# Sum02dean/GCN-STRING

Hardware: AMD Instinct MI355X
Metric: graphs/sec (fwd+bwd) on E.coli-sized batches; GCNConv SpMM achieved HBM GB/s (higher is better)
Workload: dtype f32; 1 GPU; config2: E. coli-shaped DisjointLoader batch, B=32 graphs per GPU, F=128, fp32, 2-layer GCNConv(relu)+GlobalSumPool+Dense softmax, CCE (from-logits form of tf.function), SGD; global_graphs=32, nodes_per_gpu=22576, nnz_per_gpu=333676, features=128, hidden=128, parallelism=dp1 (graphs sharded, RCCL all-reduce of 33284 fp32), hip_graph=False, gemm_precision=f32, cce=logits, activation_storage=fp32

## Files before the change

### gcn-string_amd/csrc/fused.hip

```cpp
#include "common.h"

namespace {

typedef float f32x4v __attribute__((ext_vector_type(4)));
typedef float f32x2 __attribute__((ext_vector_type(2)));
typedef __bf16 fbf16x8 __attribute__((ext_vector_type(8)));

constexpr int kFRows = 32;
constexpr int kFCap = 1024;

struct FusedArgs {
  const int32_t* rowptr; const int32_t* colidx; const float* vals;
  const float* x; int64_t ldx;
  int32_t n;
  const float* w; int32_t ldw;
  int32_t nc;
  const float* bias; int act;
  float* s; int64_t lds;
  float* wt_out;
  int w_t;
  float* out; int64_t ldo;
  const int32_t* node_graph; const int32_t* gp; const float* dp; int64_t lddp; int avg;
  const float* mask; int64_t ldmask;
  float* dz2; int64_t lddz2;
  float* colpart;
  float* tp_part; float* tp_cnt;
  const float* hd_part; const float* hd_cnt; int hd_rows; int hd_b;
  float* hd_psum; float* hd_csum;
  const float* hd_w; const float* hd_bias; const float* hd_y; int hd_c; float hd_denom; int hd_fl;
  unsigned char* m8_out; const unsigned char* m8; int64_t ldm8;
  int dbg;
};

__device__ __forceinline__ float4 fbuf4(__amdgpu_buffer_rsrc_t rs, unsigned off) {
  const f32x4v r = __builtin_bit_cast(f32x4v, __builtin_amdgcn_raw_buffer_load_b128(rs, off, 0, 0));
  return make_float4(r.x, r.y, r.z, r.w);
}
__device__ __forceinline__ float4 f4fma(float v, float4 h, float4 a) {
  const f32x2 w = {v, v};
  const f32x2 lo = __builtin_elementwise_fma(w, f32x2{h.x, h.y}, f32x2{a.x, a.y});
  const f32x2 hi = __builtin_elementwise_fma(w, f32x2{h.z, h.w}, f32x2{a.z, a.w});
  return make_float4(lo[0], lo[1], hi[0], hi[1]);
}
__device__ __forceinline__ float4 f4step(float4 a) {
  const f32x2 big = {0x1p127f, 0x1p127f};
  f32x2 lo = {a.x, a.y}, hi = {a.z, a.w}, t0, t1;
  asm("v_pk_mul_f32 %0, %1, %2" : "=v"(t0) : "v"(lo), "v"(big));
  asm("v_pk_mul_f32 %0, %1, %2" : "=v"(t1) : "v"(hi), "v"(big));
  asm("v_pk_mul_f32 %0, %1, %2 clamp" : "=v"(lo) : "v"(t0), "v"(big));
  asm("v_pk_mul_f32 %0, %1, %2 clamp" : "=v"(hi) : "v"(t1), "v"(big));
  return make_float4(lo[0], lo[1], hi[0], hi[1]);
}

constexpr int kM8B = 8;
constexpr int kM8U = 8;
typedef unsigned m8x2 __attribute__((ext_vector_type(2)));
template <int MLB> struct M8Bytes { typedef unsigned type; };
template <> struct M8Bytes<8> { typedef m8x2 type; };
template <int MLB>
__device__ __forceinline__ typename M8Bytes<MLB>::type m8load(__amdgpu_buffer_rsrc_t rs, unsigned off) {
  if constexpr (MLB == 8) return __builtin_bit_cast(m8x2, __builtin_amdgcn_raw_buffer_load_b64(rs, off, 0, 0));
  else if constexpr (MLB == 4) return (unsigned)__builtin_amdgcn_raw_buffer_load_b32(rs, off, 0, 0);
  else return (unsigned)(unsigned short)__builtin_amdgcn_raw_buffer_load_b16(rs, off, 0, 0);
}
template <int MLB>
__device__ __forceinline__ typename M8Bytes<MLB>::type m8own(const unsigned char* q) {
  if constexpr (MLB == 8) return *reinterpret_cast<const m8x2*>(q);
  else if constexpr (MLB == 4) return *reinterpret_cast<const unsigned*>(q);
  else return (unsigned)*reinterpret_cast<const unsigned short*>(q);
}
template <int MLB>
__device__ __forceinline__ unsigned m8word(typename M8Bytes<MLB>::type m, int d) {
  if constexpr (MLB == 8) return m[d]; else return m;
}
template <int MLB>
__device__ __forceinline__ void m8fma(float v, typename M8Bytes<MLB>::type m, float (&a)[MLB]) {
#pragma unroll
  for (int c = 0; c < MLB; ++c) a[c] = fmaf(v, (float)((m8word<MLB>(m, c / 4) >> (8 * (c % 4))) & 0xffu), a[c]);
}

__device__ __forceinline__ void f4acc(float4& a, const float4 q) { a.x += q.x; a.y += q.y; a.z += q.z; a.w += q.w; }

template <int LPR>
__device__ __forceinline__ float2 fused_head_dlogits(const FusedArgs& p, float4 pv, int rows, float4 w0, float4 w1, float b0,
                                                     float b1, float y0, float y1) {
  float sc = 1.0f;
  if (p.avg) { sc = 1.0f / (float)max(rows, 1); pv.x *= sc; pv.y *= sc; pv.z *= sc; pv.w *= sc; }
  const bool two = p.hd_c > 1;
  float z0 = fmaf(pv.w, w0.w, fmaf(pv.z, w0.z, fmaf(pv.y, w0.y, pv.x * w0.x)));
  float z1 = fmaf(pv.w, w1.w, fmaf(pv.z, w1.z, fmaf(pv.y, w1.y, pv.x * w1.x)));
#pragma unroll
  for (int off = 1; off < LPR; off <<= 1) { z0 += __shfl_xor(z0, off); z1 += __shfl_xor(z1, off); }
  z0 += b0;
  z1 = two ? z1 + b1 : -INFINITY;
  const float m = fmaxf(z0, z1), e0 = expf(z0 - m), e1 = expf(z1 - m), sum = e0 + e1;
  const float p0 = e0 / sum, p1 = e1 / sum;
  const bool k0 = p.hd_fl || (p0 > 1e-7f && p0 < 1.0f - 1e-7f), k1 = two && (p.hd_fl || (p1 > 1e-7f && p1 < 1.0f - 1e-7f));
  const float ymsum = (k0 ? y0 : 0.f) + (k1 ? y1 : 0.f);
  const float dl0 = (p0 * ymsum - (k0 ? y0 : 0.f)) / p.hd_denom, dl1 = two ? (p1 * ymsum - (k1 ? y1 : 0.f)) / p.hd_denom : 0.f;
  return make_float2(dl0 * sc, dl1 * sc);
}

template <int K, bool WEIGHTED, bool BWD, bool X3 = false, bool M8 = false>
__global__ __launch_bounds__(512, 6) void gcn_conv_fused_kernel(FusedArgs p) {
  constexpr int MLB = K / 16 < kM8B ? K / 16 : kM8B, UM = kM8U;
  typedef typename M8Bytes<MLB>::type m8v;
  constexpr int HL = K / 4;
  constexpr int LPR = M8 ? K / MLB : K / 4;
  constexpr int CPL = K / LPR;
  constexpr int GW = 64 / LPR;
  constexpr int NG = 8 * GW;
  constexpr int RPG = NG >= kFRows ? 1 : kFRows / NG;
  constexpr int U = 4;
  constexpr int SL = 2 * U;
  static_assert(UM <= SL, "the mask gather reads up to UM - 1 entries past a row's end");
  static_assert(K == 32 || K == 64 || K == 128, "gather width");
  static_assert(!M8 || (BWD && RPG == 1), "the byte-image gather is a backward form, one row per lane group");
  __shared__ __attribute__((aligned(16))) float tile[kFRows][K + 4];
  __shared__ __attribute__((aligned(8))) int2 s_ent[kFCap + SL];
  __shared__ int32_t s_rp[kFRows + 1];
  __shared__ unsigned char s_mb[BWD ? kFRows * 32 : 1];
  __shared__ float2 s_dl[BWD ? kFRows : 1];
  __shared__ __attribute__((aligned(16))) float s_w3[BWD ? 2 : 1][K];
  __shared__ float s_b3[2];
  __shared__ int32_t s_g[BWD ? 1 : kFRows];
  static_assert(!BWD || sizeof(float) * kFRows * (K + 4) >= sizeof(float4) * 2 * 8 * 2 * HL, "the head's wave partials alias the tile");
#ifdef GCNX_TUNING
  const int dbg = p.dbg;
#else
  constexpr int dbg = 0;
#endif

  const int tid = threadIdx.x, lane = tid & 63, wave = tid >> 6;
  const int ntiles = gridDim.x;
  const int t = gcnx_xcd_remap(blockIdx.x, ntiles);
  const int r0 = t * kFRows, nr = min(p.n - r0, kFRows);
  if (tid <= nr) s_rp[tid] = p.rowptr[r0 + tid];
  if (!BWD && p.tp_part && tid < kFRows)
    s_g[tid] = tid < nr ? min(max(p.node_graph[r0 + tid], 0), p.hd_b - 1) : -1;
  const int e0 = p.rowptr[r0], e1 = p.rowptr[r0 + nr];
  const int staged = min(e1 - e0, kFCap);
  const unsigned ld4 = M8 ? (unsigned)p.ldm8 : (unsigned)p.ldx * 4u;
  for (int i = tid; i < staged + SL; i += 512) {
    int2 en = make_int2(0, 0);
    if (i < staged) {
      en.x = (int)((unsigned)p.colidx[e0 + i] * ld4);
      en.y = WEIGHTED ? __float_as_int(p.vals[e0 + i]) : 0x3f800000;
    }
    s_ent[i] = en;
  }
  const int gid = wave * GW + lane / LPR, sub = lane % LPR;
  const __amdgpu_buffer_rsrc_t xr =
      __builtin_amdgcn_make_buffer_rsrc(M8 ? (void*)p.m8 : (void*)p.x, (short)0, (int)((unsigned)p.n * ld4), 0x00020000);
  int grow[RPG];
  if (BWD) {
#pragma unroll
    for (int j = 0; j < RPG; ++j) {
      const int r = gid + j * NG;
      grow[j] = (r < nr && gid < kFRows) ? p.node_graph[r0 + r] : -1;
    }
  }
  float4 mrow[2];
  const int mlanes = p.nc >> 2;
  if (BWD) {
#pragma unroll
    for (int q = 0; q < 2; ++q) {
      const int i = tid + 512 * q, row = i / mlanes, c4 = i - row * mlanes;
      mrow[q] = make_float4(0.f, 0.f, 0.f, 0.f);
      if (row < nr && !(dbg & 16)) mrow[q] = *reinterpret_cast<const float4*>(p.mask + (int64_t)(r0 + row) * p.ldmask + 4 * c4);
    }
  }
  float4 (*s_pv)[2][2][HL] = reinterpret_cast<float4 (*)[2][2][HL]>(&tile[0][0]);
  const int hsel = lane / HL, hsub = lane % HL;
  int g_first = 0;
  if (BWD && p.hd_part) {
    g_first = min(max(__builtin_amdgcn_readfirstlane(p.node_graph[r0]), 0), p.hd_b - 1);
    const int g_last = min(max(__builtin_amdgcn_readfirstlane(p.node_graph[r0 + nr - 1]), g_first), min(g_first + kFRows, p.hd_b) - 1);
    for (int i = tid; i < 2 * K; i += 512) {
      const int cls = i / K, k = i - cls * K;
      s_w3[cls][k] = cls < p.hd_c ? p.hd_w[(int64_t)k * p.hd_c + cls] : 0.f;
    }
    if (tid >= 2 * K && tid < 2 * K + 2) s_b3[tid - 2 * K] = (p.hd_bias && tid - 2 * K < p.hd_c) ? p.hd_bias[tid - 2 * K] : 0.f;
    const unsigned bytes = (unsigned)p.hd_rows * (unsigned)K * 4u;
    const __amdgpu_buffer_rsrc_t pr = __builtin_amdgcn_make_buffer_rsrc((void*)p.hd_part, (short)0, (int)bytes, 0x00020000);
    const __amdgpu_buffer_rsrc_t cr = __builtin_amdgcn_make_buffer_rsrc((void*)p.hd_cnt, (short)0, (int)bytes, 0x00020000);
    for (int gb = g_first; gb <= g_last; gb += 2) {
      if (gb > g_first) __syncthreads();
      int hd_g = 0, hd_n = 0;
      bool hd_desig = false;
      float y0 = 0.f, y1 = 0.f;
      if (hsel < 2) {
        hd_g = min(gb + hsel, g_last);
        const int hd_a = p.gp[hd_g];
        hd_n = p.gp[hd_g + 1] - hd_a;
        hd_desig = hd_a >= r0 && hd_n > 0;
        const int tlo = hd_a / kFRows, thi = hd_n > 0 ? (hd_a + hd_n - 1) / kFRows : tlo - 1;
        float4 ps = make_float4(0.f, 0.f, 0.f, 0.f), pc = ps;
        for (int tb = tlo + wave; __builtin_amdgcn_ballot_w64(tb <= thi) != 0; tb += 32) {
          float4 q[4], c[4];
#pragma unroll
          for (int u = 0; u < 4; ++u) {
            const int tt = tb + 8 * u;
            const unsigned off = tt <= thi ? ((unsigned)(tt + hd_g) * (unsigned)K + (unsigned)hsub * 4u) * 4u : 0xFFFFFFF0u;
            q[u] = fbuf4(pr, off);
            c[u] = fbuf4(cr, hd_desig ? off : 0xFFFFFFF0u);
          }
#pragma unroll
          for (int u = 0; u < 4; ++u) { f4acc(ps, q[u]); f4acc(pc, c[u]); }
        }
        s_pv[wave][0][hsel][hsub] = ps;
        s_pv[wave][1][hsel][hsub] = pc;
        if (wave == 0) {
          y0 = p.hd_y[(int64_t)hd_g * p.hd_c];
          y1 = p.hd_c > 1 ? p.hd_y[(int64_t)hd_g * p.hd_c + 1] : 0.f;
        }
      }
      __syncthreads();
      if (wave == 0 && hsel < 2) {
        float4 pv = make_float4(0.f, 0.f, 0.f, 0.f), pc = pv;
#pragma unroll 2
        for (int w = 0; w < 8; ++w) { f4acc(pv, s_pv[w][0][hsel][hsub]); f4acc(pc, s_pv[w][1][hsel][hsub]); }
        if (hd_desig) {
          *reinterpret_cast<float4*>(p.hd_psum + (int64_t)hd_g * K + hsub * 4) = pv;
          *reinterpret_cast<float4*>(p.hd_csum + (int64_t)hd_g * K + hsub * 4) = pc;
        }
        const float2 dl = fused_head_dlogits<HL>(p, pv, hd_n, *reinterpret_cast<const float4*>(&s_w3[0][hsub * 4]),
                                                  *reinterpret_cast<const float4*>(&s_w3[1][hsub * 4]),
                                                  s_b3[0], s_b3[1], y0, y1);
        if (hsub == 0) s_dl[hd_g - g_first] = dl;
      }
    }
  } else {
    __syncthreads();
  }
  if (BWD) {
#pragma unroll
    for (int q = 0; q < 2; ++q) {
      const int i = tid + 512 * q, row = i / mlanes, c4 = i - row * mlanes;
      if (row < kFRows)
        s_mb[row * 32 + c4] = (unsigned char)((mrow[q].x > 0.f ? 1u : 0u) | (mrow[q].y > 0.f ? 2u : 0u) | (mrow[q].z > 0.f ? 4u : 0u) |
                                              (mrow[q].w > 0.f ? 8u : 0u));
    }
  }
  float4 acc[RPG];
  int ea[RPG], eb[RPG], ebf[RPG];
  int len = 0;
#pragma unroll
  for (int j = 0; j < RPG; ++j) {
    const int r = gid + j * NG;
    acc[j] = make_float4(0.f, 0.f, 0.f, 0.f);
    const bool live = r < nr && gid < kFRows;
    ea[j] = live ? s_rp[r] - e0 : 0;
    eb[j] = live ? s_rp[r + 1] - e0 : 0;
    ebf[j] = min(eb[j], kFCap);
    ea[j] = min(ea[j], kFCap);
    len = max(len, ebf[j] - ea[j]);
  }
  if (dbg & 1) len = 0;
  const unsigned sub16 = (unsigned)sub * 16u;
  float am[M8 ? CPL : 1] = {};
  if constexpr (M8) {
    const unsigned subb = (unsigned)sub * (unsigned)MLB;
    for (int tt = 0; __builtin_amdgcn_ballot_w64(tt < len) != 0; tt += UM) {
      m8v hv[UM];
      float wv[UM];
      const int eb_ = min(ea[0] + tt, ebf[0]);
#pragma unroll
      for (int u = 0; u < UM; ++u) {
        const int e = eb_ + u;
        const int2 en = s_ent[e];
        wv[u] = __int_as_float(en.y);
        hv[u] = m8load<MLB>(xr, e < ebf[0] ? (unsigned)en.x + subb : 0xFFFFFFF0u);
      }
      __builtin_amdgcn_sched_barrier(0);
#pragma unroll
      for (int u = 0; u < UM; ++u) {
        m8fma<MLB>(wv[u], hv[u], am);
        if (u + 1 < UM) asm volatile("" : "+v"(hv[u + 1]), "+v"(am[0]));
      }
    }
    if (e1 - e0 > kFCap) {
      for (int e = max(eb[0] > 0 ? s_rp[gid] - e0 : 0, kFCap); e < eb[0]; ++e) {
        const float v = WEIGHTED ? p.vals[e0 + e] : 1.0f;
        m8fma<MLB>(v, m8load<MLB>(xr, (unsigned)p.colidx[e0 + e] * ld4 + subb), am);
      }
    }
  } else {
  for (int tt = 0; __builtin_amdgcn_ballot_w64(tt < len) != 0; tt += U) {
    float4 hv[RPG][U];
    float wv[RPG][U];
#pragma unroll
    for (int j = 0; j < RPG; ++j) {
      const int eb_ = min(ea[j] + tt, ebf[j]);
#pragma unroll
      for (int u = 0; u < U; ++u) {
        const int e = eb_ + u;
        const int2 en = s_ent[e];
        wv[j][u] = __int_as_float(en.y);
        hv[j][u] = fbuf4(xr, e < ebf[j] ? (unsigned)en.x + sub16 : 0xFFFFFFF0u);
      }
    }
    __builtin_amdgcn_sched_barrier(0);
#pragma unroll
    for (int j = 0; j < RPG; ++j)
#pragma unroll
      for (int u = 0; u < U; ++u) acc[j] = f4fma(wv[j][u], (BWD && !(dbg & 64)) ? f4step(hv[j][u]) : hv[j][u], acc[j]);
  }
  if (e1 - e0 > kFCap) {
#pragma unroll
    for (int j = 0; j < RPG; ++j)
      for (int e = max(eb[j] > 0 ? s_rp[gid + j * NG] - e0 : 0, kFCap); e < eb[j]; ++e) {
        const int c = p.colidx[e0 + e];
        const float v = WEIGHTED ? p.vals[e0 + e] : 1.0f;
        const float4 h = fbuf4(xr, (unsigned)c * ld4 + sub16);
        acc[j] = f4fma(v, BWD ? f4step(h) : h, acc[j]);
      }
  }
  }
  float4 own[RPG], dscale[RPG];
  m8v ownm = {};
  if constexpr (M8) {
    if (grow[0] >= 0 && p.dz2) ownm = m8own<MLB>(p.m8 + (int64_t)(r0 + gid) * p.ldm8 + sub * MLB);
    if (p.hd_part && !(dbg & 32)) __syncthreads();
  } else
  if (BWD) {
#pragma unroll
    for (int j = 0; j < RPG; ++j) {
      const int r = gid + j * NG;
      own[j] = dscale[j] = make_float4(0.f, 0.f, 0.f, 0.f);
      if (grow[j] >= 0 && (dbg & 32)) dscale[j] = make_float4(1.f, 1.f, 1.f, 1.f);
      if (grow[j] >= 0 && !(dbg & 32) && !p.hd_part) {
        float4 d = *reinterpret_cast<const float4*>(p.dp + (int64_t)grow[j] * p.lddp + sub * 4);
        if (p.avg) {
          const float sc = 1.0f / (float)(p.gp[grow[j] + 1] - p.gp[grow[j]]);
          d.x *= sc; d.y *= sc; d.z *= sc; d.w *= sc;
        }
        dscale[j] = d;
      }
      if (grow[j] >= 0 && p.dz2) own[j] = *reinterpret_cast<const float4*>(p.x + (int64_t)(r0 + r) * p.ldx + sub * 4);
    }
    if (p.hd_part && !(dbg & 32)) {
      __syncthreads();
      const float4 w0 = *reinterpret_cast<const float4*>(&s_w3[0][sub * 4]), w1 = *reinterpret_cast<const float4*>(&s_w3[1][sub * 4]);
#pragma unroll
      for (int j = 0; j < RPG; ++j) {
        if (grow[j] < 0) continue;
        const float2 dl = s_dl[(grow[j] - g_first) & (kFRows - 1)];
        dscale[j] = make_float4(fmaf(dl.y, w1.x, dl.x * w0.x), fmaf(dl.y, w1.y, dl.x * w0.y), fmaf(dl.y, w1.z, dl.x * w0.z),
                                fmaf(dl.y, w1.w, dl.x * w0.w));
      }
    }
  }
  const int c16 = lane & 15, kq = lane >> 4;
  const bool wave_on = 16 * wave < p.nc;
  auto k_of = [&](int e) { return X3 ? 32 * (e / 8) + 8 * kq + (e % 8) : 4 * e + kq; };
  float wreg[K / 4];
  if (wave_on && !(dbg & 4)) {
#pragma unroll
    for (int e = 0; e < K / 4; ++e)
      wreg[e] = (BWD && !p.w_t) ? p.w[(int64_t)(16 * wave + c16) * p.ldw + k_of(e)]
                                : p.w[(int64_t)k_of(e) * p.ldw + 16 * wave + c16];
    if (!BWD && p.wt_out && (int)blockIdx.x < K / 4) {
#pragma unroll
      for (int e = 0; e < K / 4; ++e)
        if (e % ntiles == (int)blockIdx.x) p.wt_out[(int64_t)(16 * wave + c16) * K + k_of(e)] = wreg[e];
    }
  }
  fbf16x8 wh[X3 ? K / 32 : 1], wl[X3 ? K / 32 : 1];
  if (X3) {
#pragma unroll
    for (int st = 0; st < K / 32; ++st)
#pragma unroll
      for (int j = 0; j < 8; ++j) {
        const float v = wave_on ? wreg[st * 8 + j] : 0.f;
        const __bf16 h = (__bf16)v;
        wh[st][j] = h;
        wl[st][j] = (__bf16)(v - (float)h);
      }
  }
  if constexpr (M8) {
    if (gid < kFRows) {
      const int r = gid, g = grow[0];
      float2 dl = make_float2(0.f, 0.f);
      float sc = 1.0f;
      if (g >= 0 && p.hd_part) dl = s_dl[(g - g_first) & (kFRows - 1)];
      else if (g >= 0 && p.avg) sc = 1.0f / (float)(p.gp[g + 1] - p.gp[g]);
      constexpr int W = CPL < 4 ? CPL : 4, NQ = CPL / W;
      const bool qs = NQ == 2 && ((sub >> 2) & 1);
      auto ldw = [](const float* q_, float (&o)[W]) {
        if constexpr (W == 4) { const float4 v = *reinterpret_cast<const float4*>(q_); o[0] = v.x; o[1] = v.y; o[2] = v.z; o[3] = v.w; }
        else { const float2 v = *reinterpret_cast<const float2*>(q_); o[0] = v.x; o[1] = v.y; }
      };
      auto stw = [](float* q_, const float (&o)[W]) {
        if constexpr (W == 4) *reinterpret_cast<float4*>(q_) = make_float4(o[0], o[1], o[2], o[3]);
        else *reinterpret_cast<float2*>(q_) = make_float2(o[0], o[1]);
      };
      float d[NQ][W];
#pragma unroll
      for (int q = 0; q < NQ; ++q) {
        const int c = sub * CPL + W * (q ^ (int)qs);
#pragma unroll
        for (int k = 0; k < W; ++k) d[q][k] = (g >= 0 && (dbg & 32)) ? 1.f : 0.f;
        if (g >= 0 && (dbg & 32)) {
        } else if (g >= 0 && p.hd_part) {
          float w0[W], w1[W];
          ldw(&s_w3[0][c], w0); ldw(&s_w3[1][c], w1);
#pragma unroll
          for (int k = 0; k < W; ++k) d[q][k] = fmaf(dl.y, w1[k], dl.x * w0[k]);
        } else if (g >= 0) {
          ldw(p.dp + (int64_t)g * p.lddp + c, d[q]);
          if (p.avg) {
#pragma unroll
            for (int k = 0; k < W; ++k) d[q][k] *= sc;
          }
        }
      }
#pragma unroll
      for (int q = 0; q < NQ; ++q) {
        const int c = sub * CPL + W * (q ^ (int)qs);
        const bool hi = NQ == 2 && ((q != 0) != qs);
        float o[W];
        if (p.dz2 && r < nr && !(dbg & 8)) {
          const unsigned ow = hi ? m8word<MLB>(ownm, NQ - 1) : m8word<MLB>(ownm, 0);
#pragma unroll
          for (int k = 0; k < W; ++k) o[k] = (float)((ow >> (8 * k)) & 0xffu) * d[q][k];
          stw(p.dz2 + (int64_t)(r0 + r) * p.lddz2 + c, o);
        }
#pragma unroll
        for (int k = 0; k < W; ++k) o[k] = (hi ? am[(NQ - 1) * W + k] : am[k]) * d[q][k];
        stw(&tile[r][c], o);
      }
    }
  } else
  if (gid < kFRows) {
#pragma unroll
    for (int j = 0; j < RPG; ++j) {
      const int r = gid + j * NG;
      float4 a = acc[j];
      if (BWD) {
        a.x *= dscale[j].x; a.y *= dscale[j].y; a.z *= dscale[j].z; a.w *= dscale[j].w;
        if (p.dz2 && r < nr && !(dbg & 8)) {
          const float4 m = f4step(own[j]);
          *reinterpret_cast<float4*>(p.dz2 + (int64_t)(r0 + r) * p.lddz2 + sub * 4) =
              make_float4(m.x * dscale[j].x, m.y * dscale[j].y, m.z * dscale[j].z, m.w * dscale[j].w);
        }
      } else if (p.s && r < nr) {
        *reinterpret_cast<float4*>(p.s + (int64_t)(r0 + r) * p.lds + sub * 4) = a;
      }
      *reinterpret_cast<float4*>(&tile[r][sub * 4]) = a;
    }
  }
  __syncthreads();
  if (!wave_on) return;
  const int col = 16 * wave + c16;
  float mk[8];
  if (BWD) {
#pragma unroll
    for (int r = 0; r < 8; ++r) {
      const int row = 16 * (r >> 2) + 4 * kq + (r & 3);
      mk[r] = (dbg & 16) ? 1.f : (float)((s_mb[row * 32 + (col >> 2)] >> (col & 3)) & 1u);
    }
  }
  const float bcol = (!BWD && p.bias) ? p.bias[col] : 0.f;
  f32x4v c0 = {0.f, 0.f, 0.f, 0.f}, c1 = c0;
  if (X3) {
    if (!(dbg & 2))
#pragma unroll
    for (int st = 0; st < K / 32; ++st) {
#pragma unroll
      for (int hf = 0; hf < 2; ++hf) {
        const float* ap = &tile[16 * hf + c16][32 * st + 8 * kq];
        const float4 x0 = *reinterpret_cast<const float4*>(ap), x1 = *reinterpret_cast<const float4*>(ap + 4);
        const float xv[8] = {x0.x, x0.y, x0.z, x0.w, x1.x, x1.y, x1.z, x1.w};
        fbf16x8 ah, al;
#pragma unroll
        for (int j = 0; j < 8; ++j) {
          const __bf16 h = (__bf16)xv[j];
          ah[j] = h;
          al[j] = (__bf16)(xv[j] - (float)h);
        }
        f32x4v& cc = hf ? c1 : c0;
        cc = __builtin_amdgcn_mfma_f32_16x16x32_bf16(ah, wl[st], cc, 0, 0, 0);
        cc = __builtin_amdgcn_mfma_f32_16x16x32_bf16(al, wh[st], cc, 0, 0, 0);
        cc = __builtin_amdgcn_mfma_f32_16x16x32_bf16(ah, wh[st], cc, 0, 0, 0);
      }
    }
  } else if (!(dbg & 2)) {
#pragma unroll
    for (int kk = 0; kk < K / 4; ++kk) {
      const float a0 = tile[c16][4 * kk + kq];
      const float a1 = tile[16 + c16][4 * kk + kq];
      c0 = __builtin_amdgcn_mfma_f32_16x16x4f32(a0, wreg[kk], c0, 0, 0, 0);
      c1 = __builtin_amdgcn_mfma_f32_16x16x4f32(a1, wreg[kk], c1, 0, 0, 0);
    }
  }
  float cs = 0.f;
  float vout[8];
#pragma unroll
  for (int r = 0; r < 8; ++r) {
    const int row = 16 * (r >> 2) + 4 * kq + (r & 3);
    float v = r < 4 ? c0[r & 3] : c1[r & 3];
    if (BWD) v = mk[r] > 0.f ? v : 0.f;
// ... 154 lines not shown
  } while (0)
  if (k == 128) GCNX_PRE_LAUNCH(128);
  else if (k == 64) GCNX_PRE_LAUNCH(64);
  else GCNX_PRE_LAUNCH(32);
#undef GCNX_PRE_LAUNCH
  GCNX_LAUNCH_OK(ctx);
  return GCNX_OK;
}

template <bool BWD>
int launch_fused(gcnx_ctx* ctx, const FusedArgs& a_in, int k, bool x3) {
  FusedArgs a = a_in;
#ifdef GCNX_TUNING
  if (const char* e = getenv("GCNX_FUSED_DBG")) a.dbg = atoi(e);
#endif
  const int tiles = gcnx_cdiv(a.n, kFRows);
  int dyn = 0;
#ifdef GCNX_TUNING
  if (const char* e = getenv("GCNX_FUSED_LDS")) dyn = atoi(e);
#endif
#define GCNX_FUSED_LAUNCH_M8(K_)                                                                                      \
  do {                                                                                                                \
    if (x3) {                                                                                                         \
      if (a.vals) hipLaunchKernelGGL((gcn_conv_fused_kernel<K_, true, BWD, true, BWD>), dim3(tiles), dim3(512), dyn, ctx->stream, a); \
      else hipLaunchKernelGGL((gcn_conv_fused_kernel<K_, false, BWD, true, BWD>), dim3(tiles), dim3(512), dyn, ctx->stream, a);      \
    } else if (a.vals) hipLaunchKernelGGL((gcn_conv_fused_kernel<K_, true, BWD, false, BWD>), dim3(tiles), dim3(512), dyn, ctx->stream, a); \
    else hipLaunchKernelGGL((gcn_conv_fused_kernel<K_, false, BWD, false, BWD>), dim3(tiles), dim3(512), dyn, ctx->stream, a);      \
  } while (0)
#define GCNX_FUSED_LAUNCH(K_)                                                                                         \
  do {                                                                                                                \
    if (x3) {                                                                                                         \
      if (a.vals) hipLaunchKernelGGL((gcn_conv_fused_kernel<K_, true, BWD, true>), dim3(tiles), dim3(512), dyn, ctx->stream, a); \
      else hipLaunchKernelGGL((gcn_conv_fused_kernel<K_, false, BWD, true>), dim3(tiles), dim3(512), dyn, ctx->stream, a);      \
    } else if (a.vals) hipLaunchKernelGGL((gcn_conv_fused_kernel<K_, true, BWD>), dim3(tiles), dim3(512), dyn, ctx->stream, a); \
    else hipLaunchKernelGGL((gcn_conv_fused_kernel<K_, false, BWD>), dim3(tiles), dim3(512), dyn, ctx->stream, a);      \
  } while (0)
  if (BWD && a.m8) {
    if (k == 128) GCNX_FUSED_LAUNCH_M8(128);
    else if (k == 64) GCNX_FUSED_LAUNCH_M8(64);
    else GCNX_FUSED_LAUNCH_M8(32);
  } else if (k == 128) GCNX_FUSED_LAUNCH(128);
  else if (k == 64) GCNX_FUSED_LAUNCH(64);
  else GCNX_FUSED_LAUNCH(32);
#undef GCNX_FUSED_LAUNCH
#undef GCNX_FUSED_LAUNCH_M8
  GCNX_LAUNCH_OK(ctx);
  return GCNX_OK;
}

inline int64_t tiles_of(int64_t n) { return (n + kFRows - 1) / kFRows; }

bool fused_shape_ok(int64_t n, int32_t k, int32_t nc, int64_t ldx) {
  return n > 0 && (k == 32 || k == 64 || k == 128) && nc >= 16 && nc <= 128 && nc % 16 == 0 && ldx >= k && ldx % 4 == 0 &&
         (uint64_t)n * (uint64_t)ldx * 4u < 0xFFFFFFF0ull;
}

}

extern "C" {

int gcnx_gcn_conv_fused_ok(int64_t n, int32_t fi, int32_t fo, int64_t ldx) { return fused_shape_ok(n, fi, fo, ldx) ? 1 : 0; }

int gcnx_gcn_conv_fwd_mask8(gcnx_ctx* ctx, const int32_t* rowptr, const int32_t* colidx, const float* vals, const float* x,
                            int64_t ldx, int32_t n, int32_t fi, const float* w, int32_t fo, const float* bias, int act, float* s,
                            int64_t lds, float* out, int64_t ldo, float* wt_out, int prec, const int32_t* node_graph, int32_t b,
                            float* tile_part, float* tile_cnt, uint8_t* mask8, int64_t ldmask8) {
  GCNX_CHECK_CTX(ctx);
  GCNX_REQUIRE(ctx, !mask8 || act == GCNX_ACT_RELU, "gcnx_gcn_conv_fwd_mask8: the byte mask is that of a ReLU output");
  GCNX_REQUIRE(ctx, !mask8 || (ldmask8 >= fo && ldmask8 % 16 == 0 && gcnx_aligned16(mask8)),
               "gcnx_gcn_conv_fwd_mask8: mask8 must be 16-byte aligned with a leading dimension in multiples of 16 bytes");
  GCNX_RANGE(ctx, "GCNConv forward (one launch)");
  GCNX_REQUIRE(ctx, (!tile_part && !tile_cnt) || (tile_part && tile_cnt && node_graph && b > 0 && gcnx_aligned16(tile_part) && gcnx_aligned16(tile_cnt)),
               "gcnx_gcn_conv_fwd_pool: the pool's partial sums need node_graph, b > 0 and two 16-byte aligned outputs");
  GCNX_REQUIRE(ctx, n >= 0 && fi >= 0 && fo >= 0, "gcnx_gcn_conv_fwd: negative size");
  if (prec != GCNX_PREC_F32 && prec != GCNX_PREC_BF16X3)
    return gcnx_fail(ctx, GCNX_ERR_UNSUPPORTED, "gcnx_gcn_conv_fwd: precision %d (GCNX_PREC_F32 or GCNX_PREC_BF16X3 here)", prec);
  GCNX_REQUIRE(ctx, act == GCNX_ACT_NONE || act == GCNX_ACT_RELU, "gcnx_gcn_conv_fwd: activation %d not supported here", act);
  if (n == 0 || fo == 0) return GCNX_OK;
  if (!fused_shape_ok(n, fi, fo, ldx))
    return gcnx_fail(ctx, GCNX_ERR_UNSUPPORTED, "gcnx_gcn_conv_fwd: needs fi in {32, 64, 128}, fo a multiple of 16 up to 128 and "
                     "n * ldx * 4 < 2^32 (got n=%d fi=%d fo=%d): use gcnx_gemm + gcnx_spmm_csr", n, fi, fo);
  GCNX_REQUIRE(ctx, rowptr && colidx && x && w && (out || mask8), "gcnx_gcn_conv_fwd: NULL pointer");
  GCNX_REQUIRE(ctx, (!out || (ldo >= fo && ldo % 4 == 0 && gcnx_aligned16(out))) && gcnx_aligned16(x) && (!bias || gcnx_aligned16(bias)) &&
                        (!s || (lds >= fi && lds % 4 == 0 && gcnx_aligned16(s))),
               "gcnx_gcn_conv_fwd: operands must be 16-byte aligned with leading dimensions in multiples of 4 floats");
  GCNX_REQUIRE(ctx, x != out && x != s, "gcnx_gcn_conv_fwd: in-place aggregation is not possible");
  FusedArgs a{};
  a.rowptr = rowptr; a.colidx = colidx; a.vals = vals; a.x = x; a.ldx = ldx; a.n = n; a.w = w; a.ldw = fo; a.nc = fo;
  a.bias = bias; a.act = act; a.s = s; a.lds = lds; a.out = out; a.ldo = ldo; a.wt_out = wt_out;
  a.node_graph = node_graph; a.tp_part = tile_part; a.tp_cnt = tile_cnt; a.hd_b = b; a.m8_out = mask8; a.ldm8 = ldmask8;
  return launch_fused<false>(ctx, a, fi, prec == GCNX_PREC_BF16X3);
}

int gcnx_gcn_conv_fwd_pool(gcnx_ctx* ctx, const int32_t* rowptr, const int32_t* colidx, const float* vals, const float* x,
                           int64_t ldx, int32_t n, int32_t fi, const float* w, int32_t fo, const float* bias, int act, float* s,
                           int64_t lds, float* out, int64_t ldo, float* wt_out, int prec, const int32_t* node_graph, int32_t b,
                           float* tile_part, float* tile_cnt) {
  return gcnx_gcn_conv_fwd_mask8(ctx, rowptr, colidx, vals, x, ldx, n, fi, w, fo, bias, act, s, lds, out, ldo, wt_out, prec,
                                 node_graph, b, tile_part, tile_cnt, nullptr, 0);
}

int gcnx_gcn_conv_fwd(gcnx_ctx* ctx, const int32_t* rowptr, const int32_t* colidx, const float* vals, const float* x,
                      int64_t ldx, int32_t n, int32_t fi, const float* w, int32_t fo, const float* bias, int act, float* s,
                      int64_t lds, float* out, int64_t ldo, float* wt_out, int prec) {
  return gcnx_gcn_conv_fwd_pool(ctx, rowptr, colidx, vals, x, ldx, n, fi, w, fo, bias, act, s, lds, out, ldo, wt_out, prec,
                                nullptr, 0, nullptr, nullptr);
}

int gcnx_gcn_conv_fwd_pre(gcnx_ctx* ctx, const float* s, int64_t lds, int32_t n, int32_t fi, const float* w, int32_t fo,
                          const float* bias, int act, float* out, int64_t ldo, int prec) {
  GCNX_CHECK_CTX(ctx);
  GCNX_RANGE(ctx, "GCNConv forward on a stored A X (one launch)");
  GCNX_REQUIRE(ctx, n >= 0 && fi >= 0 && fo >= 0, "gcnx_gcn_conv_fwd_pre: negative size");
  if (prec != GCNX_PREC_F32 && prec != GCNX_PREC_BF16X3)
    return gcnx_fail(ctx, GCNX_ERR_UNSUPPORTED, "gcnx_gcn_conv_fwd_pre: precision %d (GCNX_PREC_F32 or GCNX_PREC_BF16X3 here)", prec);
  GCNX_REQUIRE(ctx, act == GCNX_ACT_NONE || act == GCNX_ACT_RELU, "gcnx_gcn_conv_fwd_pre: activation %d not supported here", act);
  if (n == 0 || fo == 0) return GCNX_OK;
  if (!fused_shape_ok(n, fi, fo, lds))
    return gcnx_fail(ctx, GCNX_ERR_UNSUPPORTED, "gcnx_gcn_conv_fwd_pre: needs fi in {32, 64, 128}, fo a multiple of 16 up to 128, lds >= fi "
                     "in multiples of 4 floats and n * lds * 4 < 2^32 (got n=%d fi=%d fo=%d lds=%lld)", n, fi, fo, (long long)lds);
  GCNX_REQUIRE(ctx, s && w && out, "gcnx_gcn_conv_fwd_pre: NULL pointer");
  GCNX_REQUIRE(ctx, ldo >= fo && ldo % 4 == 0 && gcnx_aligned16(out) && gcnx_aligned16(s) && (!bias || gcnx_aligned16(bias)),
               "gcnx_gcn_conv_fwd_pre: operands must be 16-byte aligned with leading dimensions in multiples of 4 floats");
  GCNX_REQUIRE(ctx, s != out, "gcnx_gcn_conv_fwd_pre: out must not alias s");
  PreArgs a{};
  a.s = s; a.lds = lds; a.n = n; a.w = w; a.nc = fo; a.bias = bias; a.act = act; a.out = out; a.ldo = ldo;
  return launch_pre(ctx, a, fi, prec == GCNX_PREC_BF16X3);
}

int64_t gcnx_gcn_conv_bwd_scratch_floats(int64_t n, int32_t f1) { return n <= 0 || f1 <= 0 ? 0 : (int64_t)gcnx_cdiv(n, kFRows) * f1; }

}

namespace {

int conv_bwd_pool(gcnx_ctx* ctx, const int32_t* rowptr_t, const int32_t* colidx_t, const float* vals_t,
                           const float* y2, const uint8_t* y2m, int64_t ldy2, const int32_t* node_graph, const int32_t* graph_ptr, int32_t b,
                           const float* dpooled, int64_t lddp, int mode, int32_t n, int32_t f2, const float* w2, int32_t f1,
                           int w2_transposed, const float* y1, int64_t ldy1, float* dz2, int64_t lddz2, float* dz1, int64_t lddz1, float* db1,
                           float* scratch, int64_t scratch_floats, gcnx_pending_reduce* pending, int prec,
                           const gcnx_head_args* head) {
  GCNX_CHECK_CTX(ctx);
  GCNX_RANGE(ctx, "GCNConv backward (one launch)");
  if (prec != GCNX_PREC_F32 && prec != GCNX_PREC_BF16X3)
    return gcnx_fail(ctx, GCNX_ERR_UNSUPPORTED, "gcnx_gcn_conv_bwd_pool: precision %d (GCNX_PREC_F32 or GCNX_PREC_BF16X3 here)", prec);
  if (pending) *pending = gcnx_pending_reduce{nullptr, 0, 0, nullptr, nullptr, 0, 0, nullptr};
  GCNX_REQUIRE(ctx, n >= 0 && f1 >= 0 && f2 >= 0 && b >= 0, "gcnx_gcn_conv_bwd_pool: negative size");
  GCNX_REQUIRE(ctx, mode == GCNX_POOL_SUM || mode == GCNX_POOL_AVG,
               "gcnx_gcn_conv_bwd_pool: pool mode %d has no folded form", mode);
  if (n == 0 || f1 == 0) {
    if (db1 && f1 > 0) GCNX_HIP(ctx, hipMemsetAsync(db1, 0, (size_t)f1 * 4, ctx->stream));
    return GCNX_OK;
  }
  if (!fused_shape_ok(n, f2, f1, y2m ? f2 : ldy2) || (y2m && (ldy2 < f2 || (uint64_t)n * (uint64_t)ldy2 >= 0xFFFFFFF0ull)))
    return gcnx_fail(ctx, GCNX_ERR_UNSUPPORTED, "%s: needs f2 in {32, 64, 128}, f1 a multiple of 16 up to 128 and %s (got n=%d f1=%d f2=%d)",
                     y2m ? "gcnx_gcn_conv_bwd_pool_mask8" : "gcnx_gcn_conv_bwd_pool",
                     y2m ? "ldmask8 >= f2, n * ldmask8 < 2^32 - 16" : "n * ldy2 * 4 < 2^32", n, f1, f2);
  GCNX_REQUIRE(ctx, !y2m || ldy2 % 16 == 0, "gcnx_gcn_conv_bwd_pool_mask8: the mask's leading dimension must be a multiple of 16 bytes");
  GCNX_REQUIRE(ctx, b > 0 && rowptr_t && colidx_t && (y2 || y2m) && node_graph && graph_ptr && (dpooled || head) && w2 && y1 && dz1,
               "gcnx_gcn_conv_bwd_pool: NULL pointer");
  GCNX_REQUIRE(ctx, (head || (lddp >= f2 && lddp % 4 == 0 && gcnx_aligned16(dpooled))) && ldy1 >= f1 && ldy1 % 4 == 0 && lddz1 >= f1 &&
                        lddz1 % 4 == 0 && gcnx_aligned16(y2) && gcnx_aligned16(y2m) && gcnx_aligned16(y1) && gcnx_aligned16(dz1) &&
                        (!dz2 || (gcnx_aligned16(dz2) && lddz2 >= f2 && lddz2 % 4 == 0)),
               "gcnx_gcn_conv_bwd_pool: operands must be 16-byte aligned with leading dimensions in multiples of 4 floats");
  if (head) {
    GCNX_REQUIRE(ctx, head->tile_part && head->tile_cnt && head->pool_sum && head->pool_cnt && head->w && head->y &&
                          head->tile_rows >= tiles_of(n) + b && head->tile_rows * f2 * 4 < 0xFFFFFFF0ll && head->b == b &&
                          head->h == f2 && head->c >= 1 && head->denom > 0.f && gcnx_aligned16(head->tile_part) && gcnx_aligned16(head->tile_cnt) &&
                          gcnx_aligned16(head->pool_sum) && gcnx_aligned16(head->pool_cnt) && head->pool_mode == mode &&
                          (head->cce_mode == GCNX_CCE_PROBS || head->cce_mode == GCNX_CCE_LOGITS),
                 "gcnx_gcn_conv_bwd_pool: inconsistent head arguments");
    if (head->c > 2)
      return gcnx_fail(ctx, GCNX_ERR_UNSUPPORTED, "gcnx_gcn_conv_bwd_pool: the in-kernel head serves one or two classes (got %d)", head->c);
  }
  GCNX_REQUIRE(ctx, (y2m ? ((const void*)y2m != (const void*)dz1 && (const void*)y2m != (const void*)dz2) : (y2 != dz1 && y2 != dz2)) && y1 != dz1,
               "gcnx_gcn_conv_bwd_pool: outputs must not alias the saved activations");
  const int64_t tiles = gcnx_cdiv(n, kFRows);
  float* colpart = nullptr;
  bool defer = false;
  if (db1) {
    GCNX_REQUIRE(ctx, gcnx_aligned16(db1) && f1 % 4 == 0, "gcnx_gcn_conv_bwd_pool: db1 must be 16-byte aligned");
    defer = pending && scratch && gcnx_aligned16(scratch) && scratch_floats >= tiles * f1 && tiles <= 4096;
    if (defer) colpart = scratch;
    else {
      int rc = gcnx_ws_reserve(ctx, gcnx_colsum_partials_ws(tiles, f1));
      if (rc) return rc;
      colpart = (float*)ctx->ws;
    }
  }
  FusedArgs a{};
  a.rowptr = rowptr_t; a.colidx = colidx_t; a.vals = vals_t; a.x = y2; a.ldx = y2m ? f2 : ldy2; a.m8 = y2m; a.ldm8 = y2m ? ldy2 : 0; a.n = n; a.w = w2; a.ldw = w2_transposed ? f1 : f2; a.w_t = w2_transposed ? 1 : 0; a.nc = f1;
  a.out = dz1; a.ldo = lddz1; a.node_graph = node_graph; a.gp = graph_ptr; a.dp = dpooled; a.lddp = lddp;
  a.avg = mode == GCNX_POOL_AVG ? 1 : 0; a.mask = y1; a.ldmask = ldy1; a.dz2 = dz2; a.lddz2 = lddz2; a.colpart = colpart;
  if (head) {
    a.hd_part = head->tile_part; a.hd_cnt = head->tile_cnt; a.hd_rows = (int)head->tile_rows; a.hd_b = head->b;
    a.hd_psum = head->pool_sum; a.hd_csum = head->pool_cnt; a.hd_w = head->w; a.hd_bias = head->bias; a.hd_y = head->y;
    a.hd_c = head->c; a.hd_denom = head->denom; a.hd_fl = head->cce_mode == GCNX_CCE_LOGITS ? 1 : 0;
  }
  int rc = launch_fused<true>(ctx, a, f2, prec == GCNX_PREC_BF16X3);
  if (rc) return rc;
  if (db1) {
    if (defer) *pending = gcnx_pending_reduce{colpart, tiles, f1, db1, nullptr, 0, 0, nullptr};
    else return gcnx_colsum_partials(ctx, tiles, f1, db1);
  }
  return GCNX_OK;
}

// ... 27 lines not shown
```

Before: 386,400 graphs/s.

## Split K=128 gather rows across half-width lane groups and pack fp8 mask FMAs

For K=128 in the float path, each lane now covers two float4 halves of a row (NH=2). Lane groups shrink, so each group handles exactly one row and the multi-row-per-group loop goes away, with fewer lanes per row and more loads in flight per lane. In the mask8 weighted path, edge weights are pre-scaled and the byte mask is decoded with packed fp8-to-f32 conversions and packed FMAs. A block-wide check restages unscaled weights when any weight is too large. This adds register pressure, an extra staging pass in the rare large-weight case, and changes to offset bounds.

```diff
diff --git a/gcn-string_amd/csrc/fused.hip b/gcn-string_amd/csrc/fused.hip
--- a/gcn-string_amd/csrc/fused.hip
+++ b/gcn-string_amd/csrc/fused.hip
@@ -1,3 +1,4 @@
+#include <type_traits>
 #include "common.h"
 
 namespace {
@@ -8,6 +9,7 @@
 
 constexpr int kFRows = 32;
 constexpr int kFCap = 1024;
+constexpr unsigned kFOut = 0xFFFFFEF0u;
 
 struct FusedArgs {
   const int32_t* rowptr; const int32_t* colidx; const float* vals;
@@ -74,9 +76,23 @@
   if constexpr (MLB == 8) return m[d]; else return m;
 }
 template <int MLB>
-__device__ __forceinline__ void m8fma(float v, typename M8Bytes<MLB>::type m, float (&a)[MLB]) {
-#pragma unroll
-  for (int c = 0; c < MLB; ++c) a[c] = fmaf(v, (float)((m8word<MLB>(m, c / 4) >> (8 * (c % 4))) & 0xffu), a[c]);
+__device__ __forceinline__ void m8fma(float v, typename M8Bytes<MLB>::type m, f32x2 (&a)[MLB / 2]) {
+#pragma unroll
+  for (int c = 0; c < MLB; ++c)
+    a[c / 2][c % 2] = fmaf(v, (float)((m8word<MLB>(m, c / 4) >> (8 * (c % 4))) & 0xffu), a[c / 2][c % 2]);
+}
+constexpr float kM8One = 0x1p-9f;
+constexpr float kM8Scale = 1.0f / kM8One;
+constexpr float kM8WMax = 0x1p118f;
+template <int MLB>
+__device__ __forceinline__ void m8fma_pk(float vs, typename M8Bytes<MLB>::type m, f32x2 (&a)[MLB / 2]) {
+  const f32x2 w = {vs, vs};
+#pragma unroll
+  for (int c = 0; c < MLB / 2; ++c) {
+    const int word = (int)m8word<MLB>(m, c / 2);
+    const f32x2 f = (c & 1) ? __builtin_amdgcn_cvt_pk_f32_fp8(word, true) : __builtin_amdgcn_cvt_pk_f32_fp8(word, false);
+    a[c] = __builtin_elementwise_fma(w, f, a[c]);
+  }
 }
 
 __device__ __forceinline__ void f4acc(float4& a, const float4 q) { a.x += q.x; a.y += q.y; a.z += q.z; a.w += q.w; }
@@ -106,16 +122,19 @@
   constexpr int MLB = K / 16 < kM8B ? K / 16 : kM8B, UM = kM8U;
   typedef typename M8Bytes<MLB>::type m8v;
   constexpr int HL = K / 4;
-  constexpr int LPR = M8 ? K / MLB : K / 4;
+  constexpr int NH = (!M8 && K == 128) ? 2 : 1;
+  constexpr int LPR = M8 ? K / MLB : K / (4 * NH);
   constexpr int CPL = K / LPR;
   constexpr int GW = 64 / LPR;
   constexpr int NG = 8 * GW;
-  constexpr int RPG = NG >= kFRows ? 1 : kFRows / NG;
   constexpr int U = 4;
   constexpr int SL = 2 * U;
+  constexpr unsigned HB = (unsigned)(K / 2) * 4u;
   static_assert(UM <= SL, "the mask gather reads up to UM - 1 entries past a row's end");
   static_assert(K == 32 || K == 64 || K == 128, "gather width");
-  static_assert(!M8 || (BWD && RPG == 1), "the byte-image gather is a backward form, one row per lane group");
+  static_assert(NG >= kFRows, "one row per lane group");
+  static_assert(!M8 || BWD, "the byte-image gather is a backward form");
+  static_assert(kFOut + (NH - 1) * HB >= kFOut, "a slot past the row's end stays out of range with the immediate offset added");
   __shared__ __attribute__((aligned(16))) float tile[kFRows][K + 4];
   __shared__ __attribute__((aligned(8))) int2 s_ent[kFCap + SL];
   __shared__ int32_t s_rp[kFRows + 1];
@@ -124,6 +143,7 @@
   __shared__ __attribute__((aligned(16))) float s_w3[BWD ? 2 : 1][K];
   __shared__ float s_b3[2];
   __shared__ int32_t s_g[BWD ? 1 : kFRows];
+  __shared__ int32_t s_wbig[8];
   static_assert(!BWD || sizeof(float) * kFRows * (K + 4) >= sizeof(float4) * 2 * 8 * 2 * HL, "the head's wave partials alias the tile");
 #ifdef GCNX_TUNING
   const int dbg = p.dbg;
@@ -141,25 +161,34 @@
   const int e0 = p.rowptr[r0], e1 = p.rowptr[r0 + nr];
   const int staged = min(e1 - e0, kFCap);
   const unsigned ld4 = M8 ? (unsigned)p.ldm8 : (unsigned)p.ldx * 4u;
-  for (int i = tid; i < staged + SL; i += 512) {
-    int2 en = make_int2(0, 0);
-    if (i < staged) {
-      en.x = (int)((unsigned)p.colidx[e0 + i] * ld4);
-      en.y = WEIGHTED ? __float_as_int(p.vals[e0 + i]) : 0x3f800000;
-    }
-    s_ent[i] = en;
+  constexpr bool PK = M8 && WEIGHTED;
+  auto stage = [&](bool scaled) {
+    bool big = false;
+    for (int i = tid; i < staged + SL; i += 512) {
+      int2 en = make_int2(0, 0);
+      if (i < staged) {
+        en.x = (int)((unsigned)p.colidx[e0 + i] * ld4);
+        float wv_ = 1.0f;
+        if constexpr (WEIGHTED) {
+          wv_ = p.vals[e0 + i];
+          big |= !(fabsf(wv_) < kM8WMax);
+        }
+        en.y = __float_as_int(scaled ? wv_ * kM8Scale : wv_);
+      }
+      s_ent[i] = en;
+    }
+    return big;
+  };
+  const bool wbig = stage(M8);
+  if constexpr (PK) {
+    const bool any = __builtin_amdgcn_ballot_w64(wbig) != 0;
+    if (lane == 0) s_wbig[wave] = any ? 1 : 0;
   }
   const int gid = wave * GW + lane / LPR, sub = lane % LPR;
   const __amdgpu_buffer_rsrc_t xr =
       __builtin_amdgcn_make_buffer_rsrc(M8 ? (void*)p.m8 : (void*)p.x, (short)0, (int)((unsigned)p.n * ld4), 0x00020000);
-  int grow[RPG];
-  if (BWD) {
-#pragma unroll
-    for (int j = 0; j < RPG; ++j) {
-      const int r = gid + j * NG;
-      grow[j] = (r < nr && gid < kFRows) ? p.node_graph[r0 + r] : -1;
-    }
-  }
+  int grow = -1;
+  if (BWD && gid < nr) grow = p.node_graph[r0 + gid];
   float4 mrow[2];
   const int mlanes = p.nc >> 2;
   if (BWD) {
@@ -233,6 +262,17 @@
   } else {
     __syncthreads();
   }
+  bool plain = false;
+  if constexpr (PK) {
+    int any = 0;
+#pragma unroll
+    for (int w = 0; w < 8; ++w) any |= s_wbig[w];
+    plain = __builtin_amdgcn_readfirstlane(any) != 0;
+    if (plain) {
+      stage(false);
+      __syncthreads();
+    }
+  }
   if (BWD) {
 #pragma unroll
     for (int q = 0; q < 2; ++q) {
@@ -242,112 +282,111 @@
                                               (mrow[q].w > 0.f ? 8u : 0u));
     }
   }
-  float4 acc[RPG];
-  int ea[RPG], eb[RPG], ebf[RPG];
-  int len = 0;
-#pragma unroll
-  for (int j = 0; j < RPG; ++j) {
-    const int r = gid + j * NG;
-    acc[j] = make_float4(0.f, 0.f, 0.f, 0.f);
-    const bool live = r < nr && gid < kFRows;
-    ea[j] = live ? s_rp[r] - e0 : 0;
-    eb[j] = live ? s_rp[r + 1] - e0 : 0;
-    ebf[j] = min(eb[j], kFCap);
-    ea[j] = min(ea[j], kFCap);
-    len = max(len, ebf[j] - ea[j]);
-  }
-  if (dbg & 1) len = 0;
-  const unsigned sub16 = (unsigned)sub * 16u;
-  float am[M8 ? CPL : 1] = {};
+  const bool live = gid < nr;
+  const int eb = live ? s_rp[gid + 1] - e0 : 0;
+  const int ebf = min(eb, kFCap);
+  const int ea = min(live ? s_rp[gid] - e0 : 0, kFCap);
+  const int etail = max(eb > 0 ? s_rp[gid] - e0 : 0, kFCap);
+  const int len = (dbg & 1) ? 0 : ebf - ea;
+  float4 acc[NH];
+#pragma unroll
+  for (int h = 0; h < NH; ++h) acc[h] = make_float4(0.f, 0.f, 0.f, 0.f);
+  f32x2 am[M8 ? CPL / 2 : 1] = {};
   if constexpr (M8) {
     const unsigned subb = (unsigned)sub * (unsigned)MLB;
-    for (int tt = 0; __builtin_amdgcn_ballot_w64(tt < len) != 0; tt += UM) {
-      m8v hv[UM];
-      float wv[UM];
-      const int eb_ = min(ea[0] + tt, ebf[0]);
-#pragma unroll
-      for (int u = 0; u < UM; ++u) {
-        const int e = eb_ + u;
-        const int2 en = s_ent[e];
-        wv[u] = __int_as_float(en.y);
-        hv[u] = m8load<MLB>(xr, e < ebf[0] ? (unsigned)en.x + subb : 0xFFFFFFF0u);
-      }
-      __builtin_amdgcn_sched_barrier(0);
-#pragma unroll
-      for (int u = 0; u < UM; ++u) {
-        m8fma<MLB>(wv[u], hv[u], am);
-        if (u + 1 < UM) asm volatile("" : "+v"(hv[u + 1]), "+v"(am[0]));
-      }
-    }
+    auto gather = [&](auto pk) {
+      for (int tt = 0; __builtin_amdgcn_ballot_w64(tt < len) != 0; tt += UM) {
+        m8v hv[UM];
+        float wv[UM];
+        const int eb_ = min(ea + tt, ebf), rem = ebf - eb_;
+#pragma unroll
+        for (int u = 0; u < UM; ++u) {
+          const int2 en = s_ent[eb_ + u];
+          wv[u] = __int_as_float(en.y);
+          unsigned off = (unsigned)en.x + subb;
+          asm volatile("" : "+v"(off));
+          hv[u] = m8load<MLB>(xr, u < rem ? off : kFOut);
+        }
+        __builtin_amdgcn_sched_barrier(0);
+#pragma unroll
+        for (int u = 0; u < UM; ++u) {
+          if constexpr (decltype(pk)::value) m8fma_pk<MLB>(wv[u], hv[u], am); else m8fma<MLB>(wv[u], hv[u], am);
+          if (u + 1 < UM) asm volatile("" : "+v"(hv[u + 1]), "+v"(am[0]));
+        }
+      }
+    };
+    if (plain) gather(std::false_type{}); else gather(std::true_type{});
     if (e1 - e0 > kFCap) {
-      for (int e = max(eb[0] > 0 ? s_rp[gid] - e0 : 0, kFCap); e < eb[0]; ++e) {
+      for (int e = etail; e < eb; ++e) {
         const float v = WEIGHTED ? p.vals[e0 + e] : 1.0f;
         m8fma<MLB>(v, m8load<MLB>(xr, (unsigned)p.colidx[e0 + e] * ld4 + subb), am);
       }
     }
   } else {
-  for (int tt = 0; __builtin_amdgcn_ballot_w64(tt < len) != 0; tt += U) {
-    float4 hv[RPG][U];
-    float wv[RPG][U];
-#pragma unroll
-    for (int j = 0; j < RPG; ++j) {
-      const int eb_ = min(ea[j] + tt, ebf[j]);
+    const unsigned sub16 = (unsigned)sub * 16u;
+    for (int tt = 0; __builtin_amdgcn_ballot_w64(tt < len) != 0; tt += U) {
+      float4 hv[U][NH];
+      float wv[U];
+      const int eb_ = min(ea + tt, ebf), rem = ebf - eb_;
 #pragma unroll
       for (int u = 0; u < U; ++u) {
-        const int e = eb_ + u;
-        const int2 en = s_ent[e];
-        wv[j][u] = __int_as_float(en.y);
-        hv[j][u] = fbuf4(xr, e < ebf[j] ? (unsigned)en.x + sub16 : 0xFFFFFFF0u);
-      }
-    }
-    __builtin_amdgcn_sched_barrier(0);
-#pragma unroll
-    for (int j = 0; j < RPG; ++j)
-#pragma unroll
-      for (int u = 0; u < U; ++u) acc[j] = f4fma(wv[j][u], (BWD && !(dbg & 64)) ? f4step(hv[j][u]) : hv[j][u], acc[j]);
-  }
-  if (e1 - e0 > kFCap) {
-#pragma unroll
-    for (int j = 0; j < RPG; ++j)
-      for (int e = max(eb[j] > 0 ? s_rp[gid + j * NG] - e0 : 0, kFCap); e < eb[j]; ++e) {
-        const int c = p.colidx[e0 + e];
+        const int2 en = s_ent[eb_ + u];
+        wv[u] = __int_as_float(en.y);
+        const unsigned off = u < rem ? (unsigned)en.x + sub16 : kFOut;
+#pragma unroll
+        for (int h = 0; h < NH; ++h) hv[u][h] = fbuf4(xr, off + h * HB);
+      }
+      __builtin_amdgcn_sched_barrier(0);
+#pragma unroll
+      for (int u = 0; u < U; ++u)
+#pragma unroll
+        for (int h = 0; h < NH; ++h) acc[h] = f4fma(wv[u], (BWD && !(dbg & 64)) ? f4step(hv[u][h]) : hv[u][h], acc[h]);
+    }
+    if (e1 - e0 > kFCap) {
+      for (int e = etail; e < eb; ++e) {
+        const unsigned off = (unsigned)p.colidx[e0 + e] * ld4 + sub16;
         const float v = WEIGHTED ? p.vals[e0 + e] : 1.0f;
-        const float4 h = fbuf4(xr, (unsigned)c * ld4 + sub16);
-        acc[j] = f4fma(v, BWD ? f4step(h) : h, acc[j]);
-      }
-  }
-  }
-  float4 own[RPG], dscale[RPG];
+#pragma unroll
+        for (int h = 0; h < NH; ++h) {
+          const float4 hr = fbuf4(xr, off + h * HB);
+          acc[h] = f4fma(v, BWD ? f4step(hr) : hr, acc[h]);
+        }
+      }
+    }
+  }
+  float4 own[NH], dscale[NH];
   m8v ownm = {};
   if constexpr (M8) {
-    if (grow[0] >= 0 && p.dz2) ownm = m8own<MLB>(p.m8 + (int64_t)(r0 + gid) * p.ldm8 + sub * MLB);
+    if (grow >= 0 && p.dz2) ownm = m8own<MLB>(p.m8 + (int64_t)(r0 + gid) * p.ldm8 + sub * MLB);
     if (p.hd_part && !(dbg & 32)) __syncthreads();
   } else
   if (BWD) {
 #pragma unroll
-    for (int j = 0; j < RPG; ++j) {
-      const int r = gid + j * NG;
-      own[j] = dscale[j] = make_float4(0.f, 0.f, 0.f, 0.f);
-      if (grow[j] >= 0 && (dbg & 32)) dscale[j] = make_float4(1.f, 1.f, 1.f, 1.f);
-      if (grow[j] >= 0 && !(dbg & 32) && !p.hd_part) {
-        float4 d = *reinterpret_cast<const float4*>(p.dp + (int64_t)grow[j] * p.lddp + sub * 4);
+    for (int h = 0; h < NH; ++h) {
+      const int c = sub * 4 + h * (K / 2);
+      own[h] = dscale[h] = make_float4(0.f, 0.f, 0.f, 0.f);
+      if (grow >= 0 && (dbg & 32)) dscale[h] = make_float4(1.f, 1.f, 1.f, 1.f);
+      if (grow >= 0 && !(dbg & 32) && !p.hd_part) {
+        float4 d = *reinterpret_cast<const float4*>(p.dp + (int64_t)grow * p.lddp + c);
         if (p.avg) {
-          const float sc = 1.0f / (float)(p.gp[grow[j] + 1] - p.gp[grow[j]]);
+          const float sc = 1.0f / (float)(p.gp[grow + 1] - p.gp[grow]);
           d.x *= sc; d.y *= sc; d.z *= sc; d.w *= sc;
         }
-        dscale[j] = d;
-      }
-      if (grow[j] >= 0 && p.dz2) own[j] = *reinterpret_cast<const float4*>(p.x + (int64_t)(r0 + r) * p.ldx + sub * 4);
+        dscale[h] = d;
+      }
+      if (grow >= 0 && p.dz2) own[h] = *reinterpret_cast<const float4*>(p.x + (int64_t)(r0 + gid) * p.ldx + c);
     }
     if (p.hd_part && !(dbg & 32)) {
       __syncthreads();
-      const float4 w0 = *reinterpret_cast<const float4*>(&s_w3[0][sub * 4]), w1 = *reinterpret_cast<const float4*>(&s_w3[1][sub * 4]);
-#pragma unroll
-      for (int j = 0; j < RPG; ++j) {
-        if (grow[j] < 0) continue;
-        const float2 dl = s_dl[(grow[j] - g_first) & (kFRows - 1)];
-        dscale[j] = make_float4(fmaf(dl.y, w1.x, dl.x * w0.x), fmaf(dl.y, w1.y, dl.x * w0.y), fmaf(dl.y, w1.z, dl.x * w0.z),
-                                fmaf(dl.y, w1.w, dl.x * w0.w));
+      if (grow >= 0) {
+        const float2 dl = s_dl[(grow - g_first) & (kFRows - 1)];
+#pragma unroll
+        for (int h = 0; h < NH; ++h) {
+          const int c = sub * 4 + h * (K / 2);
+          const float4 w0 = *reinterpret_cast<const float4*>(&s_w3[0][c]), w1 = *reinterpret_cast<const float4*>(&s_w3[1][c]);
+          dscale[h] = make_float4(fmaf(dl.y, w1.x, dl.x * w0.x), fmaf(dl.y, w1.y, dl.x * w0.y), fmaf(dl.y, w1.z, dl.x * w0.z),
+                                  fmaf(dl.y, w1.w, dl.x * w0.w));
+        }
       }
     }
   }
@@ -380,7 +419,7 @@
   }
   if constexpr (M8) {
     if (gid < kFRows) {
-      const int r = gid, g = grow[0];
+      const int r = gid, g = grow;
       float2 dl = make_float2(0.f, 0.f);
       float sc = 1.0f;
       if (g >= 0 && p.hd_part) dl = s_dl[(g - g_first) & (kFRows - 1)];
@@ -427,27 +466,28 @@
           stw(p.dz2 + (int64_t)(r0 + r) * p.lddz2 + c, o);
         }
 #pragma unroll
-        for (int k = 0; k < W; ++k) o[k] = (hi ? am[(NQ - 1) * W + k] : am[k]) * d[q][k];
+        for (int k = 0; k < W; ++k) o[k] = (hi ? am[((NQ - 1) * W + k) / 2][k % 2] : am[k / 2][k % 2]) * d[q][k];
         stw(&tile[r][c], o);
       }
     }
   } else
   if (gid < kFRows) {
-#pragma unroll
-    for (int j = 0; j < RPG; ++j) {
-      const int r = gid + j * NG;
-      float4 a = acc[j];
+    const int r = gid;
+#pragma unroll
+    for (int h = 0; h < NH; ++h) {
+      const int c = sub * 4 + h * (K / 2);
+      float4 a = acc[h];
       if (BWD) {
-        a.x *= dscale[j].x; a.y *= dscale[j].y; a.z *= dscale[j].z; a.w *= dscale[j].w;
+        a.x *= dscale[h].x; a.y *= dscale[h].y; a.z *= dscale[h].z; a.w *= dscale[h].w;
         if (p.dz2 && r < nr && !(dbg & 8)) {
-          const float4 m = f4step(own[j]);
-          *reinterpret_cast<float4*>(p.dz2 + (int64_t)(r0 + r) * p.lddz2 + sub * 4) =
-              make_float4(m.x * dscale[j].x, m.y * dscale[j].y, m.z * dscale[j].z, m.w * dscale[j].w);
+          const float4 m = f4step(own[h]);
+          *reinterpret_cast<float4*>(p.dz2 + (int64_t)(r0 + r) * p.lddz2 + c) =
+              make_float4(m.x * dscale[h].x, m.y * dscale[h].y, m.z * dscale[h].z, m.w * dscale[h].w);
         }
       } else if (p.s && r < nr) {
-        *reinterpret_cast<float4*>(p.s + (int64_t)(r0 + r) * p.lds + sub * 4) = a;
-      }
-      *reinterpret_cast<float4*>(&tile[r][sub * 4]) = a;
+        *reinterpret_cast<float4*>(p.s + (int64_t)(r0 + r) * p.lds + c) = a;
+      }
+      *reinterpret_cast<float4*>(&tile[r][c]) = a;
     }
   }
   __syncthreads();
@@ -708,7 +748,7 @@
 
 bool fused_shape_ok(int64_t n, int32_t k, int32_t nc, int64_t ldx) {
   return n > 0 && (k == 32 || k == 64 || k == 128) && nc >= 16 && nc <= 128 && nc % 16 == 0 && ldx >= k && ldx % 4 == 0 &&
-         (uint64_t)n * (uint64_t)ldx * 4u < 0xFFFFFFF0ull;
+         (uint64_t)n * (uint64_t)ldx * 4u < (uint64_t)kFOut;
 }
 
 }
@@ -808,7 +848,7 @@
     if (db1 && f1 > 0) GCNX_HIP(ctx, hipMemsetAsync(db1, 0, (size_t)f1 * 4, ctx->stream));
     return GCNX_OK;
   }
-  if (!fused_shape_ok(n, f2, f1, y2m ? f2 : ldy2) || (y2m && (ldy2 < f2 || (uint64_t)n * (uint64_t)ldy2 >= 0xFFFFFFF0ull)))
+  if (!fused_shape_ok(n, f2, f1, y2m ? f2 : ldy2) || (y2m && (ldy2 < f2 || (uint64_t)n * (uint64_t)ldy2 >= (uint64_t)kFOut)))
     return gcnx_fail(ctx, GCNX_ERR_UNSUPPORTED, "%s: needs f2 in {32, 64, 128}, f1 a multiple of 16 up to 128 and %s (got n=%d f1=%d f2=%d)",
                      y2m ? "gcnx_gcn_conv_bwd_pool_mask8" : "gcnx_gcn_conv_bwd_pool",
                      y2m ? "ldmask8 >= f2, n * ldmask8 < 2^32 - 16" : "n * ldy2 * 4 < 2^32", n, f1, f2);
```

After: 388,700 graphs/s (median of 6 runs). Within noise of the previous version (+0.6%).
